# jenkinsm13/julia-spira

Measured on AMD Instinct MI355X. Metric: Msamples/sec at 1920x1080 spp=64 depth=8; fraction of HBM roofline, higher is better.
Workload: dtype f64

## Files before the change

julia-spira_amd/csrc/spira_device.h:

```cpp
#pragma once
#include <hip/hip_runtime.h>
#include <stdint.h>
#include <type_traits>
#include "spira_fastdiv.h"

namespace spira {

__device__ __forceinline__ float sqrt_rn(float x) { return __builtin_sqrtf(x); }
__device__ __forceinline__ double sqrt_rn(double x) { return __builtin_sqrt(x); }

constexpr int kBlock = 256;
#ifndef SPIRA_WAVES_F32
#define SPIRA_WAVES_F32 5
#endif
#ifndef SPIRA_WAVES_F64
#define SPIRA_WAVES_F64 4
#endif
#define SPIRA_WAVES_PER_SIMD(T) (sizeof(T) == 8 ? SPIRA_WAVES_F64 : SPIRA_WAVES_F32)
constexpr uint32_t kMaxTries = 64;

template <class T> struct Vec { T x, y, z; };

template <class T> __device__ __forceinline__ Vec<T> mk(T x, T y, T z) { Vec<T> r; r.x = x; r.y = y; r.z = z; return r; }
template <class T> __device__ __forceinline__ Vec<T> operator+(Vec<T> a, Vec<T> b) { return mk<T>(a.x + b.x, a.y + b.y, a.z + b.z); }
template <class T> __device__ __forceinline__ Vec<T> operator-(Vec<T> a, Vec<T> b) { return mk<T>(a.x - b.x, a.y - b.y, a.z - b.z); }
template <class T> __device__ __forceinline__ Vec<T> operator*(Vec<T> a, T b) { return mk<T>(a.x * b, a.y * b, a.z * b); }
template <class T> __device__ __forceinline__ Vec<T> operator/(Vec<T> a, T b) { return mk<T>(a.x / b, a.y / b, a.z / b); }
template <class T> __device__ __forceinline__ Vec<T> mulv(Vec<T> a, Vec<T> b) { return mk<T>(a.x * b.x, a.y * b.y, a.z * b.z); }
template <class T> __device__ __forceinline__ T dot(Vec<T> a, Vec<T> b) { return a.x * b.x + a.y * b.y + a.z * b.z; }
template <class T> __device__ __forceinline__ Vec<T> cross(Vec<T> a, Vec<T> b) {
    return mk<T>(a.y * b.z - a.z * b.y, a.z * b.x - a.x * b.z, a.x * b.y - a.y * b.x);
}
__device__ __forceinline__ float abs_t(float x) { return __builtin_fabsf(x); }
__device__ __forceinline__ double abs_t(double x) { return __builtin_fabs(x); }
template <class T> __device__ __forceinline__ Vec<T> normalize(Vec<T> a) { return a / sqrt_rn(dot(a, a)); }

struct ExactDiv {};
// ... 691 lines not shown
            oc = o - mk<T>(c.x, c.y, c.z);
            cc = dot(oc, oc) - c.w;
        }
        T b = (T)2.0 * dot(oc, d);
        const T bb = b * b;
        T disc = bb - four_a * cc;
        if (!(disc < 0)) {
            root_operands<T>(bb, disc, pol);
            T sq = root_sqrt<T>(disc, pol);
            T root = root_over<T>(-b - sq, over_2a, pol);
            bool ok = !(root < t_min || root > closest);
            if (!ok && root < t_min) {
                root = root_over<T>(-b + sq, over_2a, pol);
                ok = !(root < t_min || root > closest);
            }
            if (ok) { closest = root; prim = (int)s; }
        }
    }
    if (TRI && sc.n_triangles) {
        Pack4<T> v0n = sc.tri[0], e1n = sc.tri[1], e2n = sc.tri[2];
#pragma unroll 2
        for (uint32_t i = 0; i < sc.n_triangles; ++i) {
            const Pack4<T> v0 = v0n, e1 = e1n, e2 = e2n;
            const uint32_t nx = i + 1 < sc.n_triangles ? i + 1 : i;
            v0n = sc.tri[3 * nx]; e1n = sc.tri[3 * nx + 1]; e2n = sc.tri[3 * nx + 2];
            T t;
            if (triangle_test<T>(v0, e1, e2, o, d, t_min, closest, t, pol)) {
                closest = t; prim = (int)(sc.n_spheres + i);
            }
        }
    }
}

template <class T>
__device__ __forceinline__ bool mesh_box_hit(const SceneLds<T> &sc, Vec<T> o, Vec<T> d, T closest) {
    const Vec<T> inv = mk<T>(rcp_fast(d.x), rcp_fast(d.y), rcp_fast(d.z));
    return box_entry<T>(sc.bvh_root[0], sc.bvh_root[1], o, inv, closest) >= (T)0;
}

template <class T>
__device__ __forceinline__ void closest_hit_local(const SceneLds<T> &sc, Vec<T> o, Vec<T> d, T t_min, T &closest, int &prim) {
    ExactDiv exact;
    closest_hit_local<T>(sc, o, d, t_min, closest, prim, exact);
}
template <class T, bool BVH, class P, bool TRI = true>
__device__ __forceinline__ int closest_hit(const SceneLds<T> &sc, Vec<T> o, Vec<T> d, T t_min, T &t_hit, uint32_t &slot, P &pol) {
    T closest; int prim;
    closest_hit_local<T, P, TRI>(sc, o, d, t_min, closest, prim, pol);
    slot = 0;
    if (BVH) bvh_closest_hit<T>(sc, o, d, t_min, closest, prim, slot);
    t_hit = closest;
    return prim;
}
template <class T, bool BVH>
__device__ __forceinline__ int closest_hit(const SceneLds<T> &sc, Vec<T> o, Vec<T> d, T t_min, T &t_hit, uint32_t &slot) {
    ExactDiv exact;
    return closest_hit<T, BVH>(sc, o, d, t_min, t_hit, slot, exact);
}

template <class T> __device__ __forceinline__ Vec<T> random_in_unit_sphere(const RngKey &k) {
    Vec<T> p = mk<T>(0, 0, 0);
    for (uint32_t t = 1; t <= kMaxTries; ++t) {
        T u0, u1, u2;
        rng3<T>(k, t, u0, u1, u2, (T)(1.0 / 1048576.0));
        Vec<T> q = mk<T>(u0, u1, u2) - mk<T>(1, 1, 1);
        if (dot(q, q) < (T)1.0) { p = q; break; }
// ... 174 lines not shown
                                           Vec<T> &o, Vec<T> &d, P &pol) {
    T xu, xv, unused;
    rng3<T>(rng_key(rc.sA, rc.sB, pixel, sample, 0), 0, xu, xv, unused);
    T u = ((T)(i - 1) + xu) / (T)(rc.width - 1);
    T v = ((T)(j - 1) + xv) / (T)(rc.height - 1);
    o = rc.cam_origin;
    d = normalize(((rc.cam_llc + rc.cam_hor * u) + rc.cam_ver * v) - o, pol);
}
template <class T>
__device__ __forceinline__ void camera_ray(const RenderConst<T> &rc, uint32_t i, uint32_t j, uint32_t pixel, uint32_t sample,
                                           Vec<T> &o, Vec<T> &d) {
    ExactDiv exact;
    camera_ray<T>(rc, i, j, pixel, sample, o, d, exact);
}
__device__ __forceinline__ float to_scalar(float x) { return __uint_as_float(__builtin_amdgcn_readfirstlane(__float_as_uint(x))); }
__device__ __forceinline__ double to_scalar(double x) {
    const uint32_t lo = __builtin_amdgcn_readfirstlane((uint32_t)__double2loint(x)), hi = __builtin_amdgcn_readfirstlane((uint32_t)__double2hiint(x));
    return __hiloint2double((int)hi, (int)lo);
}
template <class T> struct PixelDiv { Recip<T> w1, h1; };
template <class T> __device__ __forceinline__ PixelDiv<T> pixel_divisors(const RenderConst<T> &rc) {
    PixelDiv<T> p;
    p.w1 = recip_of((T)(rc.width - 1)); p.h1 = recip_of((T)(rc.height - 1));
    p.w1.d = to_scalar(p.w1.d); p.w1.r = to_scalar(p.w1.r); p.h1.d = to_scalar(p.h1.d); p.h1.r = to_scalar(p.h1.r);
    return p;
}
template <class T> __device__ __forceinline__ T pixel_quotient(T n, const Recip<T> &rc, ExactDiv &) { return n / rc.d; }
template <class T> __device__ __forceinline__ T pixel_quotient(T n, const Recip<T> &rc, SpecDiv &) { return quotient(n, rc); }
template <class T, class P>
__device__ __forceinline__ void camera_ray_lds(const RenderConst<T> &rc, const T *cam, const PixelDiv<T> &pd, uint32_t i, uint32_t j, uint32_t pixel, uint32_t sample,
                                               Vec<T> &o, Vec<T> &d, P &pol) {
    T xu, xv, unused;
    rng3<T>(rng_key(rc.sA, rc.sB, pixel, sample, 0), 0, xu, xv, unused);
    T u = pixel_quotient<T>((T)(i - 1) + xu, pd.w1, pol);
    T v = pixel_quotient<T>((T)(j - 1) + xv, pd.h1, pol);
    o = mk<T>(cam[0], cam[1], cam[2]);
    const Vec<T> llc = mk<T>(cam[3], cam[4], cam[5]), hor = mk<T>(cam[6], cam[7], cam[8]), ver = mk<T>(cam[9], cam[10], cam[11]);
    d = normalize(((llc + hor * u) + ver * v) - o, pol);
}

template <class T>
__device__ __forceinline__ void path_of(const RenderConst<T> &rc, uint32_t q, uint32_t pass, uint32_t &i, uint32_t &j,
                                        uint32_t &pixel, uint32_t &sample) {
    uint32_t slot = fastdiv(q, rc.fd_tile);
    uint32_t pl = q - slot * rc.tile_pixels;
    uint32_t lr = fastdiv(pl, rc.fd_width);
    uint32_t lx = pl - lr * rc.width;
    j = ref_row_j(rc, lr);
    i = lx + 1;
    pixel = (j - 1) * rc.width + lx;
    sample = rc.sample0 + pass * rc.slots + slot;
}

template <class T> struct RayQueue { Pack4<T> *A; Pack4<T> *B; Pack2<T> *C; };

struct Stats {
    unsigned long long segments, rays_enqueued, radiance_rmw, radiance_store, redone_waves, rays_parked;
    unsigned long long mesh_wave_trips, mesh_lane_trips;
};

template <class T> struct BounceArgs {
    SceneGlobal<T> scene;
    RenderConst<T> rc;
    RayQueue<T> qin, qout;
    Pack3<T> *L;
    const uint32_t *cnt_in;
// ... 245 lines not shown
        a.blk_stats[4 * wid + 1] = n_rmw;
        a.blk_stats[4 * wid + 2] = n_store;
        a.blk_stats[4 * wid + 3] = FIRST ? 0u : n_seg;
    }
}

template <class T> struct PathArgs {
    SceneGlobal<T> scene;
    RenderConst<T> rc;
    RayQueue<T> q[2];
    uint32_t *qref[2];
    uint2 *qkey[2];
    uint32_t cam_consts;
    Pack3<T> *L;
    uint32_t *blk_stats;
    uint32_t cap;
    uint32_t pass;
    uint32_t n_first;
    uint32_t dense_pct;
    Pack4<T> *mesh_list;
    uint32_t mesh_min_batch;
    uint32_t refill_free;
    uint32_t mesh_mode;
    uint32_t *mesh_count;
    uint32_t resume_k, resume_nw;
    uint32_t *redo;
    uint32_t redo_only;
    Stats *stats;
    Pack4<T> *accum;
    FastDiv fd_keff;
    uint32_t k_eff;
    uint32_t accum_first;
    uint32_t l_private;
};

#ifndef SPIRA_RESOLVE_RUN
#define SPIRA_RESOLVE_RUN 4
#endif
__device__ __forceinline__ uint32_t owned_pixel(uint32_t w, uint32_t nw, uint32_t l) {
    constexpr uint32_t kRun = SPIRA_RESOLVE_RUN;
    static_assert(64 % kRun == 0, "a run length divides the wave");
    return ((l / kRun) * nw + w) * kRun + l % kRun;
}

template <class T>
__device__ __forceinline__ void resolve_pixel(Pack4<T> *accum, const Pack3<T> *L, uint32_t tile_pixels, uint32_t k_eff, bool first_pass, uint32_t p) {
    Pack4<T> acc;
    if (first_pass) { acc.x = 0; acc.y = 0; acc.z = 0; acc.w = 0; } else acc = accum[p];
    uint32_t s = 0;
    for (; s + 8 <= k_eff; s += 8) {
        Pack3<T> l[8];
#pragma unroll
        for (int k = 0; k < 8; ++k) l[k] = L[(size_t)(s + k) * tile_pixels + p];
#pragma unroll
        for (int k = 0; k < 8; ++k) { acc.x = acc.x + l[k].x; acc.y = acc.y + l[k].y; acc.z = acc.z + l[k].z; }
    }
    for (; s < k_eff; ++s) {
        const Pack3<T> l = L[(size_t)s * tile_pixels + p];
        acc.x = acc.x + l.x; acc.y = acc.y + l.y; acc.z = acc.z + l.z;
    }
    accum[p] = acc;
}
template <class T>
__device__ __forceinline__ void resolve_pixel_run(Pack4<T> *accum, const Pack3<T> *Lp, uint32_t k_eff, bool first_pass, uint32_t p) {
    constexpr uint32_t kRun = SPIRA_RESOLVE_RUN;
    Pack4<T> acc;
    if (first_pass) { acc.x = 0; acc.y = 0; acc.z = 0; acc.w = 0; } else acc = accum[p];
// ... 64 lines not shown
    constexpr bool kCam = !EXT;
    if (kCam && MODE != 2 && a.cam_consts)
        for (uint32_t i = threadIdx.x; i < a.scene.n_spheres; i += blockDim.x) {
            const T *sp = a.scene.spheres5 + 5 * (size_t)i;
            const Vec<T> oc = rc.cam_origin - mk<T>(sp[0], sp[1], sp[2]);
            Pack4<T> k; k.x = oc.x; k.y = oc.y; k.z = oc.z; k.w = dot(oc, oc) - sp[3] * sp[3];
            cam_sph[i] = k;
        }
    const SceneLds<T> sc = stage_scene<T>(a.scene, lds_raw);
    const PixelDiv<T> pix_div = pixel_divisors<T>(rc);
    if (!SPEC && a.redo_only) {
        if (!a.redo[wid]) return;
        if (lane == 0) atomicAdd(&a.stats->redone_waves, 1ull);
    }
    Pack4<T> *s_rnd = reinterpret_cast<Pack4<T> *>(lds_raw + scene_lds_bytes<T>(a.scene.n_spheres, a.scene.n_materials, a.scene.n_triangles)) + wave * SUB;
    constexpr uint32_t mesh_mode = BVH ? (uint32_t)MODE : 0u;
    const uint32_t kseg = mesh_mode == 2u ? a.resume_k : 1u;
    if (mesh_mode == 2u && wid * kseg >= a.resume_nw) return;
    const uint32_t region = wid * kseg * a.cap;
    const unsigned long long lt_mask = (1ull << lane) - 1ull;
    const uint32_t ref_base = sc.n_spheres + sc.n_triangles;
    const bool mixed = mesh_mode != 0u || rc.max_depth <= 128u;
    const uint32_t dense_pct = mixed ? a.dense_pct : 0u;
    const bool defer = mesh_mode != 0u || (BVH && mixed && a.mesh_list != nullptr);
    Pack4<T> *mlist = a.mesh_list + 3 * (size_t)region;
    uint32_t n_rmw = 0, n_store = 0, n_seg = 0, n_enq = 0, n_park = 0;
    uint32_t n_wtrips = 0, n_ltrips = 0;
    uint32_t n_in = 0;
    const bool own = !BVH && !EXT && !TRI && sizeof(T) == 8 && a.accum != nullptr;
    const uint32_t n_own = own ? 64u * a.k_eff : 0u;
    const uint32_t n_sub_first = own ? (n_own + SUB - 1) / SUB : (a.n_first + SUB - 1) / SUB;
    const bool priv = kCarry && own && a.l_private != 0;
    const uint32_t l_base = priv ? wid * n_own : 0u;

    auto park = [&](uint32_t slot_i, const Vec<T> o_, const Vec<T> d_, const Vec<T> beta_, T closest_, uint32_t q_, int prim_, uint32_t stage_hit) {
        Pack4<T> A, B, C;
        A.x = o_.x; A.y = o_.y; A.z = o_.z; A.w = d_.x;
        B.x = d_.y; B.y = d_.z; B.z = beta_.x; B.w = beta_.y;
        C.x = beta_.z; C.y = closest_; C.z = Bits<T>::from_u32(q_); C.w = Bits<T>::from_u32((uint32_t)(prim_ + 1) | (stage_hit << kStageShift));
        mlist[3 * (size_t)slot_i] = A; mlist[3 * (size_t)slot_i + 1] = B; mlist[3 * (size_t)slot_i + 2] = C;
    };
    uint32_t mfill = 0;
    constexpr int kMaxSeg = 16;
    uint32_t pfx[kMaxSeg + 1];
    bool segmented = false;
    {
        uint32_t cnt = 0;
        if (mesh_mode == 2u && lane < kseg && wid * kseg + lane < a.resume_nw) cnt = a.mesh_count[wid * kseg + lane];
        pfx[0] = 0;
#pragma unroll
        for (int j = 0; j < kMaxSeg; ++j) pfx[j + 1] = pfx[j] + (uint32_t)__builtin_amdgcn_readlane((int)cnt, j);
        if (mesh_mode == 2u) { mfill = pfx[kMaxSeg]; segmented = true; }
    }
    const uint32_t first_sub = own ? 0u : (mesh_mode == 1u ? (wid % a.resume_k) * (NW / a.resume_k) + wid / a.resume_k : wid);
    const uint32_t sub_step = own ? 1u : NW;
    MESH_STAT(unsigned long long dbg_t0 = __builtin_readcyclecounter(); unsigned long long dbg_sess = 0, dbg_walk = 0; uint32_t dbg_ns = 0, dbg_ws = 0, dbg_ls = 0, dbg_rf = 0, dbg_rays = 0, dbg_rounds = 0, dbg_ws1 = 0, dbg_ls1 = 0, dbg_h[4] = {0, 0, 0, 0};)
    for (uint32_t round = 0; ; ++round) {
        MESH_STAT(++dbg_rounds;)
        const bool first = mesh_mode != 2u && round == 0;
        const RayQueue<T> qin = a.q[(round + 1) & 1], qout = a.q[round & 1];
        const uint32_t *rin = a.qref[(round + 1) & 1];
        uint32_t *rout = a.qref[round & 1];
        const uint2 *kin = a.qkey[(round + 1) & 1];
        uint2 *kout = a.qkey[round & 1];
        const uint32_t limit = first ? (own ? n_own : a.n_first) : n_in;
        const uint32_t n_sub = first ? n_sub_first : (n_in + SUB - 1) / SUB;
        uint32_t fill = 0;
        for (uint32_t sub = first ? first_sub : 0u; sub < n_sub; sub += first ? sub_step : 1u) {
            Vec<T> o[R], beta[R];
            Pending<T> pend[R];
            ExtState<T> ex[R];
            uint32_t q[R], ent[R], stg[R], ref[R];
            uint32_t ka[R], kb[R];
            bool valid[R];
#pragma unroll
            for (int r = 0; r < R; ++r) {
                const uint32_t idx = sub * SUB + r * 64 + lane;
                valid[r] = false; stg[r] = round; ref[r] = 0; q[r] = 0; ka[r] = 0; kb[r] = 0;
                pend[r].kind = kDead; pend[r].rough = 0; pend[r].v = mk<T>(0, 0, 0);
                o[r] = mk<T>(0, 0, 0); beta[r] = mk<T>(1, 1, 1);
                bool parked = false; T park_t = 0; int park_prim = -1;
                uint32_t qf = idx;
                bool in = idx < limit;
                if (own && first) {
                    const uint32_t t = idx / SPIRA_RESOLVE_RUN, run = fastdiv(t, a.fd_keff);
                    const uint32_t px = owned_pixel(wid, NW, run * SPIRA_RESOLVE_RUN + idx % SPIRA_RESOLVE_RUN);
                    qf = (t - run * a.k_eff) * rc.tile_pixels + px;
                    in = in && px < rc.tile_pixels;
                }
                const uint32_t ql = priv ? l_base + idx : qf;
                if (in) {
                    if (first) {
                        uint32_t pixel, sample, pi, pj;
                        Vec<T> d;
                        q[r] = ql;
                        path_of<T>(rc, qf, a.pass, pi, pj, pixel, sample);
                        if (kCarry) { ka[r] = mix32(rc.sA + pixel) ^ (sample << 8); kb[r] = mix32(rc.sB ^ pixel) + (sample << 8); }
                        camera_ray_lds<T>(rc, cam_lds, pix_div, pi, pj, pixel, sample, o[r], d, pol);
                        if (EXT) { ex[r].flags = rc.flags; if (rc.flags & kExtSpectral) beta[r] = ext_wavelength<T>(sc, rc.sA, rc.sB, pixel, sample, ex[r]); }
                        T t; uint32_t slot = 0;
                        int prim;
                        if (defer) {
                            if (kCam && a.cam_consts) closest_hit_local<T, Pol, TRI, true>(sc, o[r], d, (T)0.001, t, prim, pol, cam_sph);
                            else closest_hit_local<T, Pol, TRI>(sc, o[r], d, (T)0.001, t, prim, pol);
                            parked = mesh_box_hit<T>(sc, o[r], d, t);
                        } else if (kCam && !BVH && a.cam_consts) { closest_hit_local<T, Pol, TRI, true>(sc, o[r], d, (T)0.001, t, prim, pol, cam_sph); }
                        else prim = closest_hit<T, BVH, Pol, TRI>(sc, o[r], d, (T)0.001, t, slot, pol);
                        ++n_seg;
                        if (parked) { park_t = t; park_prim = prim; pend[r].v = d; }
                        else if (prim < 0) {
                            const Vec<T> c = sky_term_x<T, EXT>(d, beta[r], &ex[r]);
                            Pack3<T> l; l.x = c.x; l.y = c.y; l.z = c.z;
                            a.L[ql] = l;
                            ++n_store;
                        } else {
                            valid[r] = true;
                            o[r] = o[r] + d * t;
                            ref[r] = (BVH && prim >= (int)ref_base) ? ref_base + slot : (uint32_t)prim;
                            pend[r].v = d;
                        }
                    } else {
                        const Pack4<T> A = qin.A[region + idx], B = qin.B[region + idx];
                        const Pack2<T> C = qin.C[region + idx];
                        o[r] = mk<T>(A.x, A.y, A.z);
                        pend[r].v = mk<T>(A.w, B.x, B.y);
                        beta[r] = mk<T>(B.z, B.w, C.x);
                        q[r] = unpack_q(C.y);
                        uint32_t w;
                        if constexpr (kRefArray) w = rin[region + idx]; else w = unpack_ref(C.y);
                        if (mixed) { stg[r] = w >> kStageShift; ref[r] = w & kRefMask; } else ref[r] = w;
                        if (kCarry) { const uint2 k = kin[region + idx]; ka[r] = k.x; kb[r] = k.y; }
                        valid[r] = true;
                    }
                }
                if (defer && first) {
// ... 1199 lines not shown
```

julia-spira_amd/csrc/spira_hip.hip:

```cpp
#include <hip/hip_runtime.h>
#include <sys/mman.h>
#include <rccl/rccl.h>
#include <dlfcn.h>

#include <algorithm>
#include <atomic>
#include <chrono>
#include <cmath>
#include <cstdio>
#include <cstdlib>
#include <cstring>
#include <condition_variable>
#include <mutex>
#include <new>
#include <string>
#include <thread>
#include <vector>

#include "../../include/spira_hip.h"
#include "../../include/spira_spd.h"
#include "spira_device.h"
#include "spira_bvh.h"
#include "spira_validate.h"
#include "spira_plan.h"
// ... 534 lines not shown
        static_assert(SPIRA_SPD_N == spira::kSpdN && SPIRA_SPD_ROWS == spira::kSpdRows, "SPD table shape");
        T host[SPIRA_SPD_ROWS * SPIRA_SPD_N];
        for (int r = 0; r < SPIRA_SPD_ROWS; ++r)
            for (int i = 0; i < SPIRA_SPD_N; ++i) host[r * SPIRA_SPD_N + i] = (T)spira_spd_table[r][i];
        if (int rc = b.ensure(sizeof host)) return rc;
        HIP_TRY(hipMemcpy(b.p, host, sizeof host, hipMemcpyHostToDevice));
    }
    (void)st;
    g.spd = (const T *)b.p;
    return 0;
}

template <class T>
int check_handle(const spira_scene *h) {
    if (!h || h->magic != kSceneMagic) return fail(SPIRA_E_INVALID, "scene handle is NULL or was destroyed");
    if (h->prec != (int)sizeof(T)) return fail(SPIRA_E_INVALID, "scene handle was created in the other precision");
    if (h->device != tl_device) return fail(SPIRA_E_INVALID, "scene handle belongs to another device (spira_set_device)");
    return 0;
}

spira::Knobs read_knobs() {
    spira::Knobs k;
    k.batch_rays = env_u32("SPIRA_BATCH_RAYS", k.batch_rays);
    k.R = env_u32("SPIRA_R", k.R);
    k.blocks_per_cu = env_u32("SPIRA_BLOCKS_PER_CU", 0);
    k.defer_mesh = env_u32("SPIRA_DEFER_MESH", 1); k.mesh_two_pass = env_u32("SPIRA_MESH_TWO_PASS", 1);
    k.fused_resolve = env_u32("SPIRA_FUSED_RESOLVE", 1); k.private_l = env_u32("SPIRA_PRIVATE_L", 1);
    k.spec_div = env_u32("SPIRA_SPEC_DIV", 1);
    k.dense_pct = std::min<uint32_t>(env_u32("SPIRA_DENSE_PCT", 70), 100);
    k.mesh_min_batch = std::max<uint32_t>(1, env_u32("SPIRA_MESH_MIN_BATCH", 128));
    k.mesh_refill = std::min<uint32_t>(64, std::max<uint32_t>(1, env_u32("SPIRA_MESH_REFILL", 16)));
    k.mesh_fat_waves_per_cu = env_u32("SPIRA_MESH_FAT_WAVES_PER_CU", 16);
    k.cam_consts = env_u32("SPIRA_CAM_CONSTS", 1);
    return k;
}
template <class T>
spira::PlanIn plan_input(const Ctx &c, const spira_params *p, uint32_t rows, uint32_t nt_scene, bool progressive, bool caller_rng, bool out_on_device) {
    spira::PlanIn in;
    in.width = p->width; in.rows = rows; in.spp = p->spp; in.max_depth = p->max_depth; in.flags = p->flags; in.batch_rays = p->batch_rays;
    in.n_triangles = nt_scene; in.num_cus = (uint32_t)c.num_cus;
    in.progressive = progressive; in.caller_rng = caller_rng; in.out_on_device = out_on_device;
    in.prec = sizeof(T); in.block = spira::kBlock; in.waves_per_simd = SPIRA_WAVES_PER_SIMD(T); in.carry_key = SPIRA_CARRY_KEY;
    in.pack4 = sizeof(spira::Pack4<T>); in.pack3 = sizeof(spira::Pack3<T>); in.pack2 = sizeof(spira::Pack2<T>);
    in.k = read_knobs();
    return in;
}

int ensure_workspaces(Ctx &c, const spira::Workspace &w) {
    for (int i = 0; i < 2; ++i) {
        if (int rc = c.qA[i].ensure(w.queue4)) return rc;
        if (int rc = c.qB[i].ensure(w.queue4)) return rc;
        if (int rc = c.qC[i].ensure(w.queue2)) return rc;
        if (int rc = c.qR[i].ensure(w.q_ref)) return rc;
        if (int rc = c.qK[i].ensure(w.q_key)) return rc;
        if (int rc = c.qX[i].ensure(w.q_x)) return rc;
    }
    const struct { DevBuf &b; uint64_t bytes; } rest[] = {
        {c.mesh_list, w.mesh_list}, {c.mesh_count, w.mesh_count}, {c.redo, w.redo}, {c.blkstats, w.blkstats}, {c.L, w.L}, {c.counts, w.counts},
        {c.stats, sizeof(spira::Stats)}, {c.accum, w.accum}, {c.out_tmp, w.out_tmp}, {c.rng, w.rng},
        {c.hyb_state, w.hyb_state}, {c.hyb_mat, w.hyb_mat}, {c.hyb_flags, w.hyb_flags}};
    for (const auto &r : rest)
        if (int rc = r.b.ensure(r.bytes)) return rc;
    return 0;
}

template <class T>
int verify_path_args(const Ctx &c, const spira::PathArgs<T> &a, uint32_t first_launch_blocks) {
    using P4 = spira::Pack4<T>;
    using P2 = spira::Pack2<T>;
    spira::PathLaunch l;
    l.blocks = first_launch_blocks; l.cap = a.cap; l.n_first = a.n_first; l.k_eff = a.k_eff;
    l.tile_pixels = a.rc.tile_pixels; l.max_depth = a.rc.max_depth; l.flags = a.rc.flags; l.n_lds_triangles = a.scene.n_triangles;
    l.mesh_mode = a.mesh_mode; l.resume_k = a.resume_k; l.resume_nw = a.resume_nw;
    l.mesh = a.scene.n_bvh_tris != 0; l.pixel_owning = a.accum != nullptr; l.l_private = a.l_private != 0;
    l.prec = sizeof(T); l.wpb = spira::kBlock / 64; l.carry_key = SPIRA_CARRY_KEY;
    const spira::PathNeed need = spira::path_need(l);
    const uint64_t nw = need.nw, n = need.packets;
    auto covers = [](const DevBuf &b, const void *ptr, uint64_t bytes) { return ptr == b.p && b.p != nullptr && b.cap >= bytes; };
    const char *bad = need.fits ? nullptr : "the pass does not fit its queue regions";
    if (a.rc.max_depth > 1 || l.mesh)
        for (int i = 0; i < 2 && !bad; ++i) {
            if (!covers(c.qA[i], a.q[i].A, n * sizeof(P4)) || !covers(c.qB[i], a.q[i].B, n * sizeof(P4)) || !covers(c.qC[i], a.q[i].C, n * sizeof(P2))) bad = "hit queues";
            else if (sizeof(T) == 4 && !covers(c.qR[i], a.qref[i], n * sizeof(uint32_t))) bad = "hit reference arrays";
            else if (!l.mesh && !covers(c.qK[i], a.qkey[i], n * sizeof(uint2))) bad = "carried RNG keys";
        }
    if (!bad && a.mesh_list && !covers(c.mesh_list, a.mesh_list, 3 * n * sizeof(P4))) bad = "mesh lists";
    if (!bad && a.mesh_mode != 0 && (!a.mesh_list || !covers(c.mesh_count, a.mesh_count, nw * sizeof(uint32_t)) || !need.resume_ok)) bad = "parked-ray counts of a two-launch mesh pass";
    if (!bad && a.redo && !covers(c.redo, a.redo, nw * sizeof(uint32_t))) bad = "redo flags";
    if (!bad && !covers(c.blkstats, a.blk_stats, nw * 4 * sizeof(uint32_t))) bad = "per-wave statistics";
    if (!bad && !covers(c.L, a.L, need.l_entries * sizeof(spira::Pack3<T>))) bad = "per-path radiance";
    if (!bad && !covers(c.stats, a.stats, sizeof(spira::Stats))) bad = "counters";
    if (!bad && a.accum && (!covers(c.accum, a.accum, (uint64_t)a.rc.tile_pixels * sizeof(P4)) || !need.owning_ok)) bad = "pixel-owning pass";
    if (!bad && a.l_private && !need.private_ok) bad = "wave-private radiance blocks";
    if (bad) return fail(SPIRA_E_LIMIT, std::string("internal: a workspace is smaller than the launch needs (") + bad + ")");
    return 0;
}

template <class T>
int validate_call(const spira_scene *h, const T *spheres5, const T *materials8, const T *triangles10, const T *camera12, const spira_params *p,
                  const T *out_hdr, const T *out_img, bool progressive, uint32_t sample0, const uint32_t *rng_states, uint32_t *rows) {
    if (!p) return fail(SPIRA_E_INVALID, "params is NULL");
    const uint32_t nt = triangles10 ? p->n_triangles : 0;
    if (h) { if (int rc = check_handle<T>(h)) return rc; }
    else if (int rc = validate_scene<T>(spheres5, materials8, triangles10, p->n_spheres, p->n_materials, nt)) return rc;
    if (int rc = validate_params(camera12, p, h ? h->store.nt : nt, rows)) return rc;
    if (!out_hdr && !out_img) return fail(SPIRA_E_INVALID, "both outputs are NULL");
    const char *msg = nullptr;
    if (int rc = spira::sample_range_check(progressive, sample0, p->spp, &msg)) return fail(rc, msg);
    if (progressive && (p->flags & SPIRA_SEM_MASK) == SPIRA_SEM_HYBRID) return fail(SPIRA_E_UNSUPPORTED, "SPIRA_SEM_HYBRID has no accumulate entry (its image is a mean of tone-mapped samples)");
    if (progressive && (p->flags & SPIRA_SEM_MASK) == SPIRA_SEM_METAL && sample0 > 0 && !rng_states)
        return fail(SPIRA_E_INVALID, "SPIRA_SEM_METAL with sample0 > 0 needs rng_states (the LCG states the previous call left); "
                                     "without them every call would replay the samples of the first");
    return 0;
}

template <class T> struct Call {
    Ctx &c;
    hipStream_t st;
    const spira_params *p;
    const spira::Plan &plan;
    spira::BounceArgs<T> a{};
    size_t lds = 0;
    int spec = 0;
    bool progressive = false, profile = false;
    uint32_t sample0 = 0, *d_rng = nullptr;
    uint64_t launches = 0, metal_launches = 0;
// ... 105 lines not shown
    const spira::Plan &plan = k.plan;
    const spira::Knobs &kn = plan.in.k;
    spira::PathArgs<T> pa{};
    pa.scene = k.a.scene; pa.rc = k.a.rc; pa.L = k.a.L; pa.pass = k.a.pass; pa.n_first = k.a.n_first;
    pa.dense_pct = kn.dense_pct;
    pa.mesh_list = plan.defer_mesh ? (P4 *)c.mesh_list.p : nullptr;
    const spira::Geometry g = plan.geometry(pa.n_first);
    const uint32_t G = g.G;
    pa.cap = g.cap;
    *stat_rows = G * plan.wpb;
    for (int i = 0; i < 2; ++i) {
        pa.q[i] = k.queue(i);
        pa.qref[i] = (uint32_t *)c.qR[i].p;
        pa.qkey[i] = (uint2 *)c.qK[i].p;
    }
    pa.blk_stats = (uint32_t *)c.blkstats.p;
    pa.stats = k.stats();
    if (k.spec) pa.redo = k.redo();
    pa.mesh_mode = 0; pa.mesh_count = nullptr; pa.resume_k = 1; pa.resume_nw = 0;
    pa.mesh_min_batch = kn.mesh_min_batch;
    pa.refill_free = kn.mesh_refill;
    size_t lds_a = k.lds + (size_t)plan.wpb * plan.sub * sizeof(P4) + 128;
    pa.cam_consts = (kn.cam_consts && pa.scene.n_spheres && lds_a + (size_t)pa.scene.n_spheres * sizeof(P4) <= (size_t)160 * 1024) ? 1u : 0u;
    if (pa.cam_consts) lds_a += (size_t)pa.scene.n_spheres * sizeof(P4);
    if (plan.two_pass) {
        pa.mesh_mode = 1; pa.mesh_count = (uint32_t *)c.mesh_count.p;
        pa.resume_nw = G * plan.wpb; pa.resume_k = plan.fat_k(pa.resume_nw);
    }
    if (plan.fused) {
        pa.accum = k.accum(); pa.k_eff = plan.k_eff(pa.pass); pa.fd_keff = spira::fastdiv_make(pa.k_eff);
        pa.accum_first = (pa.pass == 0 && !k.progressive) ? 1u : 0u;
        pa.l_private = plan.l_private ? 1u : 0u;
    }
    if (int rc = verify_path_args<T>(c, pa, G)) return rc;
    HIP_TRY(hipEventRecord(c.ev_pool[c.ev_used++], k.st));
    if (int rc = launch_path<T>((int)plan.R, dim3(G), lds_a, k.st, pa, k.spec)) return rc;
    if (int rc = lds_optin_failed()) return rc;
    k.launches += k.spec ? 2 : 1;
    if (pa.mesh_mode == 1) {
        if (c.ev_mid.size() <= c.ev_mid_used) {
            hipEvent_t e;
            HIP_TRY(hipEventCreate(&e));
            c.ev_mid.push_back(e); c.ev_mid_end.push_back(0);
        }
        HIP_TRY(hipEventRecord(c.ev_mid[c.ev_mid_used], k.st));
        c.ev_mid_end[c.ev_mid_used++] = c.ev_used;
        spira::PathArgs<T> pb = pa;
        pb.mesh_mode = 2; pb.n_first = 0;
        const uint32_t nwb = pa.resume_nw / pa.resume_k;
        launch_path_resume_entry<T>((int)plan.R, dim3((nwb + plan.wpb - 1) / plan.wpb), lds_a, k.st, pb);
        if (int rc = lds_optin_failed()) return rc;
        ++k.launches;
    }
    HIP_TRY(hipEventRecord(c.ev_pool[c.ev_used++], k.st));
    return 0;
}

template <class T>
int enqueue_bounce_pass(Call<T> &k, uint32_t *stat_rows) {
    using P4 = typename Call<T>::P4;
    Ctx &c = k.c;
    const spira::Plan &plan = k.plan;
    const spira::Geometry g = plan.geometry(k.a.n_first);
    const size_t nw = (size_t)g.G * plan.wpb;
    k.a.cap = g.cap;
    *stat_rows = k.p->max_depth * g.G * plan.wpb;
    for (uint32_t b = 0; b < k.p->max_depth; ++b) {
// ... 1247 lines not shown
```

julia-spira_amd/csrc/spira_plan.h:

```cpp
#pragma once
#include <algorithm>
#include <cstdint>

#include "../../include/spira_hip.h"

namespace spira {

struct Knobs {
    uint32_t batch_rays = 160u << 20;
    uint32_t R = 2;
    uint32_t blocks_per_cu = 0;
    uint32_t defer_mesh = 1, mesh_two_pass = 1, fused_resolve = 1, private_l = 1;
    uint32_t spec_div = 1;
    uint32_t dense_pct = 70, mesh_min_batch = 128, mesh_refill = 16, mesh_fat_waves_per_cu = 16, cam_consts = 1;
};

struct PlanIn {
    uint32_t width = 0, rows = 0;
    uint32_t spp = 0, max_depth = 0, flags = 0, batch_rays = 0;
    uint32_t n_triangles = 0;
    uint32_t num_cus = 0;
    bool progressive = false, caller_rng = false, out_on_device = false;
    bool adaptive = false;
    uint32_t prec = 0, block = 0, waves_per_simd = 0, carry_key = 0;
    uint32_t pack4 = 0, pack3 = 0, pack2 = 0;
    Knobs k;
};

enum class Org { Black, Hybrid, MetalWavefront, Metal, Cpu, Mega, Path, Bounce };

struct Geometry { uint32_t G, cap; };

struct Workspace {
    uint64_t queue4 = 0, queue2 = 0, q_ref = 0, q_key = 0, q_x = 0;
    uint64_t mesh_list = 0, mesh_count = 0, redo = 0, blkstats = 0, L = 0, counts = 0, accum = 0, out_tmp = 0, rng = 0;
    uint64_t hyb_state = 0, hyb_mat = 0, hyb_flags = 0;
};

struct Plan {
    PlanIn in;
    Org org = Org::Black;
    uint32_t R = 2, wpb = 0, sub = 0, max_blocks = 0;
    uint64_t tile_pixels = 0, batch = 0;
    uint32_t slots = 0, n_pass = 0;
    bool mesh_scene = false, defer_mesh = false, two_pass = false;
    bool fused = false, l_private = false;
    bool spec_allowed = false;
    uint32_t G_max = 0, cap_max = 0;
    uint64_t q_rays = 0;
    uint32_t ppw = 0, G_metal = 0;
    Workspace ws;

    Geometry geometry(uint64_t n_first) const {
        if (fused) {
            const uint64_t k = n_first / tile_pixels;
            return {(uint32_t)((tile_pixels + 64 * wpb - 1) / (64 * wpb)), (uint32_t)((64 * k + sub - 1) / sub * sub)};
        }
        const uint64_t n_sub = (n_first + sub - 1) / sub;
        const uint32_t G = (uint32_t)std::min<uint64_t>((n_sub + wpb - 1) / wpb, max_blocks);
        const uint64_t nw = (uint64_t)G * wpb;
        return {G, (uint32_t)(((n_sub + nw - 1) / nw) * sub)};
    }
    uint32_t k_eff(uint32_t pass) const { return std::min(slots, in.spp - pass * slots); }
    uint32_t n_first(uint32_t pass) const { return (uint32_t)((uint64_t)k_eff(pass) * tile_pixels); }
    uint32_t blocks(uint64_t n) const { return (uint32_t)std::min<uint64_t>((n + in.block - 1) / in.block, max_blocks); }
    uint32_t fat_k(uint32_t nw) const {
        const uint32_t fat = std::max<uint32_t>(1, in.num_cus * in.k.mesh_fat_waves_per_cu);
        uint32_t k = 16;
        while (k > 1 && (nw % k != 0 || nw / k < fat)) k >>= 1;
        return k;
    }
    int spec(bool moderate) const {
        uint32_t s = spec_allowed ? in.k.spec_div : 0;
        if (s == 1 && !moderate) s = 0;
        return s > 2 ? 1 : (int)s;
    }
};

inline int sample_range_check(bool progressive, uint32_t sample0, uint32_t spp, const char **msg) {
    if (progressive && (uint64_t)sample0 + spp > SPIRA_MAX_SPP) { *msg = "sample0 + spp exceeds 2^24"; return SPIRA_E_LIMIT; }
    return 0;
}

inline int make_plan(const PlanIn &in, Plan &pl, const char **msg) {
    auto bad = [&](const char *m) { *msg = m; return SPIRA_E_LIMIT; };
    pl = Plan{};
    pl.in = in;
    const Knobs &k = in.k;
    const uint32_t sem = in.flags & SPIRA_SEM_MASK, kern = in.flags & SPIRA_KERNEL_MASK;
    const bool ext = (in.flags & (SPIRA_EXT_DIELECTRIC | SPIRA_EXT_SPECTRAL)) != 0;
    const uint64_t tp = pl.tile_pixels = (uint64_t)in.rows * in.width;
    const uint32_t target = in.batch_rays ? in.batch_rays : k.batch_rays;
    uint64_t slots = std::min<uint64_t>(std::max<uint64_t>(1, target / tp), in.spp);
    const uint64_t n_pass = (in.spp + slots - 1) / slots;
    slots = (in.spp + n_pass - 1) / n_pass;
    if (slots * tp > 0x7FFFFFFFull) return bad("tile too large: rows*width must be < 2^31");
    pl.slots = (uint32_t)slots;
    pl.n_pass = (in.spp + pl.slots - 1) / pl.slots;
    pl.batch = slots * tp;
    pl.org = sem == SPIRA_SEM_HYBRID ? Org::Hybrid : sem == SPIRA_SEM_METAL ? (kern == SPIRA_KERNEL_WAVEFRONT ? Org::MetalWavefront : Org::Metal) :
             sem == SPIRA_SEM_CPU ? Org::Cpu : kern == SPIRA_KERNEL_MEGA ? Org::Mega : kern == SPIRA_KERNEL_BOUNCE ? Org::Bounce : Org::Path;
    const bool persistent = pl.org == Org::Path;
    pl.R = (k.R == 1 && !ext) ? 1 : 2;
    pl.mesh_scene = in.n_triangles > SPIRA_LDS_TRIANGLES;
    pl.defer_mesh = persistent && pl.mesh_scene && in.max_depth <= 128 && k.defer_mesh != 0;
    pl.two_pass = pl.defer_mesh && k.mesh_two_pass != 0;

    const uint32_t blocks_per_cu = k.blocks_per_cu ? k.blocks_per_cu : !persistent ? 16 : (pl.mesh_scene && !pl.two_pass) ? 4 : 32;
    pl.max_blocks = (uint32_t)std::min<uint64_t>((uint64_t)in.num_cus * blocks_per_cu, 0x7FFFFFFFull);
    pl.wpb = in.block / 64;
    pl.sub = 64 * pl.R;
    pl.fused = persistent && in.prec == 8 && pl.R == 2 && in.n_triangles == 0 && !ext && pl.slots <= 64 && k.fused_resolve != 0 && !in.adaptive;
    const Geometry g = pl.geometry(pl.batch);
    pl.G_max = g.G; pl.cap_max = g.cap;
    const uint64_t waves = (uint64_t)g.G * pl.wpb;
    pl.l_private = pl.fused && in.carry_key && in.max_depth <= 128 && k.private_l != 0 && 64ull * waves * pl.slots <= 0x7FFFFFFFull;
    pl.q_rays = (uint64_t)g.cap * waves;
    if (pl.q_rays > 0xFFFFFFFFull) return bad("pass too large");
    pl.spec_allowed = pl.org == Org::Cpu || (pl.org == Org::Metal && !in.progressive) || (pl.org == Org::MetalWavefront && !in.progressive && pl.R == 2) ||
                      (persistent && pl.R == 2);
    if (in.max_depth == 0) pl.org = Org::Black;

    Workspace &w = pl.ws;
    const uint64_t redo_per_wave = (pl.spec_allowed && k.spec_div) ? sizeof(uint32_t) : 0, stat_row = 4 * sizeof(uint32_t);
    w.accum = tp * in.pack4;
    w.out_tmp = in.out_on_device ? 0 : 2 * 3 * tp * in.prec;
    if (in.caller_rng && !in.out_on_device) w.rng = tp * sizeof(uint32_t);
    switch (pl.org) {
    case Org::Black: break;
    case Org::Hybrid:
        if (tp > 0xFFFFFFFFull / 2) return bad("image too large for SPIRA_SEM_HYBRID");
        w.hyb_state = 12 * tp * in.prec; w.hyb_mat = w.rng = tp * sizeof(uint32_t);
        w.hyb_flags = (uint64_t)in.spp * (in.max_depth + 1) * sizeof(uint32_t);
        break;
    case Org::MetalWavefront: {
        const uint64_t nw0 = (uint64_t)in.num_cus * in.waves_per_simd * pl.wpb;
        pl.ppw = (uint32_t)((((tp + nw0 - 1) / nw0) + 63) / 64 * 64);
        pl.G_metal = (uint32_t)((tp + (uint64_t)pl.ppw * pl.wpb - 1) / ((uint64_t)pl.ppw * pl.wpb));
        const uint64_t nw = (uint64_t)pl.G_metal * pl.wpb, n = nw * pl.ppw;
        w.queue4 = n * in.pack4; w.queue2 = n * in.pack2; w.q_x = n * 2 * sizeof(uint32_t); w.L = n * in.pack3;
        if (!in.caller_rng) w.rng = tp * sizeof(uint32_t);
        w.blkstats = nw * stat_row; w.redo = nw * redo_per_wave;
        break;
    }
    case Org::Metal: case Org::Cpu: case Org::Mega:
        w.L = pl.batch * in.pack3; w.blkstats = waves * stat_row;
        w.redo = (pl.org == Org::Metal ? pl.blocks(tp) : pl.org == Org::Cpu ? pl.max_blocks : 0) * (uint64_t)pl.wpb * redo_per_wave;
        break;
    case Org::Bounce:
        if (in.max_depth > 1) { w.queue4 = pl.q_rays * in.pack4; w.queue2 = pl.q_rays * in.pack2; }
        w.L = pl.batch * in.pack3;
        w.counts = (uint64_t)(in.max_depth + 2) * waves * sizeof(uint32_t); w.blkstats = (uint64_t)(in.max_depth + 1) * waves * stat_row;
        break;
    case Org::Path:
        if (in.max_depth > 1 || pl.mesh_scene) {
            w.queue4 = pl.q_rays * in.pack4; w.queue2 = pl.q_rays * in.pack2;
            if (in.prec == 4) w.q_ref = pl.q_rays * sizeof(uint32_t);
            if (!pl.defer_mesh) w.q_key = pl.q_rays * 2 * sizeof(uint32_t);
        }
        if (pl.defer_mesh) w.mesh_list = 3 * pl.q_rays * in.pack4;
        if (pl.two_pass) w.mesh_count = waves * sizeof(uint32_t);
        w.redo = waves * redo_per_wave; w.blkstats = waves * stat_row;
        w.L = (pl.l_private ? std::max<uint64_t>(pl.batch, 64ull * waves * pl.slots) : pl.batch) * in.pack3;
        break;
    }
    return 0;
}

struct PathLaunch {
    uint32_t blocks = 0, cap = 0, n_first = 0, k_eff = 0;
    uint32_t tile_pixels = 0, max_depth = 0, flags = 0, n_lds_triangles = 0;
    uint32_t mesh_mode = 0, resume_k = 1, resume_nw = 0;
    bool mesh = false, pixel_owning = false, l_private = false;
    uint32_t prec = 0, wpb = 0, carry_key = 0;
};
struct PathNeed {
    uint64_t nw, packets, l_entries;
    bool fits, resume_ok, owning_ok, private_ok;
};
inline PathNeed path_need(const PathLaunch &a) {
    PathNeed n{};
    n.nw = (uint64_t)a.blocks * a.wpb;
    n.packets = n.nw * a.cap;
    n.fits = a.n_first <= n.packets;
    n.resume_ok = a.resume_k != 0 && a.resume_k <= 16 && n.nw % a.resume_k == 0 && a.resume_nw == n.nw;
    n.l_entries = a.l_private ? std::max<uint64_t>(a.n_first, 64ull * n.nw * a.k_eff) : a.n_first;
    const uint64_t tp = a.tile_pixels;
    n.owning_ok = a.prec == 8 && !a.n_lds_triangles && !a.mesh && !(a.flags & (SPIRA_EXT_DIELECTRIC | SPIRA_EXT_SPECTRAL)) && a.k_eff != 0 && a.k_eff <= 64 &&
                  (uint64_t)a.k_eff * tp == a.n_first && 64 * n.nw >= tp && a.cap >= 64ull * a.k_eff;
    n.private_ok = a.pixel_owning && a.carry_key && a.max_depth <= 128 && n.l_entries <= 0x80000000ull;
    return n;
}

struct AdaptiveIn {
    uint32_t min_spp = 0, batch_spp = 0, spp = 0;
    double tolerance = 0, floor = 0;
    uint64_t tile_pixels = 0;
    uint32_t prec = 0, pack3 = 0, num_cus = 0;
};
constexpr uint32_t kAdaptiveItems = 256, kAdaptiveWpb = 4;
struct AdaptiveRound { uint32_t samples, chunk, ppw, grid; uint64_t waves; };
struct AdaptivePlan {
    AdaptiveIn in;
    uint32_t levels = 0;
    uint64_t list_cap = 0;
    uint64_t list_bytes = 0, q_bytes = 0, n_bytes = 0, count_bytes = 0;
    uint64_t lds_round = 0;
    uint32_t level(uint32_t r) const { return (uint32_t)std::min<uint64_t>((uint64_t)in.min_spp + (uint64_t)r * in.batch_spp, in.spp); }
    AdaptiveRound round(uint32_t r, uint64_t n_active) const {
        AdaptiveRound a{};
        a.samples = level(r) - level(r - 1);
        a.chunk = std::min(a.samples, kAdaptiveItems);
        const uint64_t want_waves = std::max<uint64_t>(1, (uint64_t)in.num_cus * 16);
        const uint64_t spread = (n_active + want_waves - 1) / want_waves;
        a.ppw = (uint32_t)std::max<uint64_t>(1, std::min<uint64_t>(std::min<uint32_t>(64, kAdaptiveItems / a.chunk), spread));
        a.waves = (n_active + a.ppw - 1) / a.ppw;
        a.grid = (uint32_t)((a.waves + kAdaptiveWpb - 1) / kAdaptiveWpb);
        return a;
    }
};
inline int adaptive_check(uint32_t min_spp, uint32_t batch_spp, uint32_t spp, double tolerance, double floor, const char **msg) {
    if (min_spp < 2) { *msg = "spira_adaptive: min_spp must be >= 2 (a variance needs two samples)"; return SPIRA_E_INVALID; }
    if (batch_spp < 1) { *msg = "spira_adaptive: batch_spp must be >= 1"; return SPIRA_E_INVALID; }
// ... 85 lines not shown
```

Measured before the change: 28160.

## Add per-wave LDS pixel table and camera-ray sphere culling masks

In the fused pixel-owning f64 path, each wave precomputes per-lane pixel coordinates and RNG hash constants into an LDS table. This removes the repeated path_of divisions and hashing for every primary ray. It also builds a conservative per-pixel-footprint bitmask of spheres that camera rays could hit, and primary rays test only those spheres. The cost is extra LDS per block, a setup loop over spheres per lane, and the risk that a culling bound that is not conservative enough drops hits.

```diff
diff --git a/julia-spira_amd/csrc/spira_cam_cull.h b/julia-spira_amd/csrc/spira_cam_cull.h
--- /dev/null
+++ b/julia-spira_amd/csrc/spira_cam_cull.h
@@ -0,0 +1,40 @@
+#pragma once
+#include <math.h>
+#include <stdint.h>
+#if defined(__HIPCC__)
+#define SPIRA_CULL_HD __host__ __device__
+#else
+#define SPIRA_CULL_HD
+#endif
+
+namespace spira {
+
+constexpr uint32_t kPixelTableEntry = 16, kPixelTableWave = 64 * kPixelTableEntry + 64 * 8;
+constexpr uint32_t kCamCullMaxSpheres = 64;
+
+SPIRA_CULL_HD inline bool cam_sphere_culled(const double *cam, uint32_t W, uint32_t H, uint32_t pi, uint32_t pj, const double *pk) {
+    if (W < 2 || H < 2) return false;
+    const double kMargin = 1.0 / 1073741824.0;
+    const double ocx = pk[0], ocy = pk[1], ocz = pk[2];
+    const double oc2 = ocx * ocx + ocy * ocy + ocz * ocz;
+    const double slack = kMargin * oc2;
+    if (!(pk[3] > slack)) return false;
+    const double r2 = oc2 - pk[3];
+    const double w1 = (double)(W - 1), h1 = (double)(H - 1);
+    const double uc = ((double)pi - 0.5) / w1, vc = ((double)pj - 0.5) / h1;
+    const double hu = 0.5 / w1, hv = 0.5 / h1;
+    const double dcx = (cam[3] + cam[6] * uc + cam[9] * vc) - cam[0];
+    const double dcy = (cam[4] + cam[7] * uc + cam[10] * vc) - cam[1];
+    const double dcz = (cam[5] + cam[8] * uc + cam[11] * vc) - cam[2];
+    const double rho = hu * sqrt(cam[6] * cam[6] + cam[7] * cam[7] + cam[8] * cam[8]) + hv * sqrt(cam[9] * cam[9] + cam[10] * cam[10] + cam[11] * cam[11]);
+    const double cx = ocy * dcz - ocz * dcy, cy = ocz * dcx - ocx * dcz, cz = ocx * dcy - ocy * dcx;
+    const double N = sqrt(cx * cx + cy * cy + cz * cz) - sqrt(oc2) * rho;
+    const double M = sqrt(dcx * dcx + dcy * dcy + dcz * dcz) + rho;
+    if (!(N > 0)) return false;
+    const double lhs = N * N, rhs = (r2 + slack) * (M * M);
+    if (!(lhs > rhs)) return false;
+    const double fin = lhs + rhs;
+    return fin - fin == 0;
+}
+
+}
diff --git a/julia-spira_amd/csrc/spira_device.h b/julia-spira_amd/csrc/spira_device.h
--- a/julia-spira_amd/csrc/spira_device.h
+++ b/julia-spira_amd/csrc/spira_device.h
@@ -3,6 +3,7 @@
 #include <stdint.h>
 #include <type_traits>
 #include "spira_fastdiv.h"
+#include "spira_cam_cull.h"
 
 namespace spira {
 
@@ -760,6 +761,43 @@
     }
 }
 
+template <class T, class P>
+__device__ __forceinline__ void closest_hit_cam_masked(Vec<T> d, T t_min, T &closest, int &prim, P &pol, const Pack4<T> *cam, unsigned long long mask) {
+    closest = (T)INFINITY;
+    prim = -1;
+    const T a = dot(d, d);
+    const T two_a = (T)2.0 * a;
+    const T four_a = (T)4 * a;
+    const RootDiv<T> over_2a = root_divisor<T>(two_a, pol);
+    root_t_min<T>(t_min, pol);
+    if (!mask) return;
+    uint32_t s_next = (uint32_t)__builtin_ctzll(mask);
+    mask &= mask - 1ull;
+    Pack4<T> c_next = cam[s_next];
+    while (true) {
+        const Pack4<T> c = c_next;
+        const uint32_t s = s_next;
+        const bool more = mask != 0;
+        if (more) { s_next = (uint32_t)__builtin_ctzll(mask); mask &= mask - 1ull; c_next = cam[s_next]; }
+        const Vec<T> oc = mk<T>(c.x, c.y, c.z);
+        T b = (T)2.0 * dot(oc, d);
+        const T bb = b * b;
+        T disc = bb - four_a * c.w;
+        if (!(disc < 0)) {
+            root_operands<T>(bb, disc, pol);
+            T sq = root_sqrt<T>(disc, pol);
+            T root = root_over<T>(-b - sq, over_2a, pol);
+            bool ok = !(root < t_min || root > closest);
+            if (!ok && root < t_min) {
+                root = root_over<T>(-b + sq, over_2a, pol);
+                ok = !(root < t_min || root > closest);
+            }
+            if (ok) { closest = root; prim = (int)s; }
+        }
+        if (!more) break;
+    }
+}
+
 template <class T>
 __device__ __forceinline__ bool mesh_box_hit(const SceneLds<T> &sc, Vec<T> o, Vec<T> d, T closest) {
     const Vec<T> inv = mk<T>(rcp_fast(d.x), rcp_fast(d.y), rcp_fast(d.z));
@@ -1000,6 +1038,19 @@
                                                Vec<T> &o, Vec<T> &d, P &pol) {
     T xu, xv, unused;
     rng3<T>(rng_key(rc.sA, rc.sB, pixel, sample, 0), 0, xu, xv, unused);
+    T u = pixel_quotient<T>((T)(i - 1) + xu, pd.w1, pol);
+    T v = pixel_quotient<T>((T)(j - 1) + xv, pd.h1, pol);
+    o = mk<T>(cam[0], cam[1], cam[2]);
+    const Vec<T> llc = mk<T>(cam[3], cam[4], cam[5]), hor = mk<T>(cam[6], cam[7], cam[8]), ver = mk<T>(cam[9], cam[10], cam[11]);
+    d = normalize(((llc + hor * u) + ver * v) - o, pol);
+}
+template <class T, class P>
+__device__ __forceinline__ void camera_ray_lds(const T *cam, const PixelDiv<T> &pd, uint32_t i, uint32_t j, uint32_t mA, uint32_t mB, uint32_t sample,
+                                               Vec<T> &o, Vec<T> &d, P &pol) {
+    T xu, xv, unused;
+    RngKey k;
+    k.hA = mix32(mA ^ (sample << 8)); k.hB = mix32(mB + (sample << 8)); k.hBr = (k.hB << 16) | (k.hB >> 16);
+    rng3<T>(k, 0, xu, xv, unused);
     T u = pixel_quotient<T>((T)(i - 1) + xu, pd.w1, pol);
     T v = pixel_quotient<T>((T)(j - 1) + xv, pd.h1, pol);
     o = mk<T>(cam[0], cam[1], cam[2]);
@@ -1311,7 +1362,9 @@
     uint32_t k_eff;
     uint32_t accum_first;
     uint32_t l_private;
+    uint32_t pixel_table;
 };
+constexpr uint32_t kTableConsts = 1u, kTableCull = 2u;
 
 #ifndef SPIRA_RESOLVE_RUN
 #define SPIRA_RESOLVE_RUN 4
@@ -1442,6 +1495,38 @@
     const uint32_t n_sub_first = own ? (n_own + SUB - 1) / SUB : (a.n_first + SUB - 1) / SUB;
     const bool priv = kCarry && own && a.l_private != 0;
     const uint32_t l_base = priv ? wid * n_own : 0u;
+    constexpr bool kOwn = !BVH && !EXT && !TRI && sizeof(T) == 8 && R == 2 && MODE == 0;
+    uint32_t tab_bits = 0;
+    const uint4 *ptab = nullptr;
+    const uint2 *pmask = nullptr;
+    if constexpr (kOwn) {
+        if (own && a.pixel_table) {
+            constexpr uint32_t kRun = SPIRA_RESOLVE_RUN;
+            tab_bits = a.pixel_table;
+            unsigned char *tb = reinterpret_cast<unsigned char *>(cam_sph + (a.cam_consts ? a.scene.n_spheres : 0u)) +
+                                (uint32_t)__builtin_amdgcn_readfirstlane((int)wave) * kPixelTableWave;
+            uint4 *tab_w = reinterpret_cast<uint4 *>(tb);
+            uint2 *mask_w = reinterpret_cast<uint2 *>(tb + 64 * kPixelTableEntry);
+            const uint32_t px = owned_pixel(wid, NW, lane);
+            uint4 e = make_uint4(0u, 0u, 0u, 0u);
+            unsigned long long m = 0;
+            if (px < rc.tile_pixels) {
+                uint32_t pi, pj, pixel, sample;
+                path_of<T>(rc, px, a.pass, pi, pj, pixel, sample);
+                e = make_uint4(pi, pj, mix32(rc.sA + pixel), mix32(rc.sB ^ pixel));
+                if (tab_bits & kTableCull)
+                    for (uint32_t s = 0; s < a.scene.n_spheres; ++s)
+                        if (!cam_sphere_culled(cam_lds, rc.width, rc.height, pi, pj, &cam_sph[s].x)) m |= 1ull << s;
+            }
+            uint32_t lo = (uint32_t)m, hi = (uint32_t)(m >> 32);
+#pragma unroll
+            for (uint32_t dl = 1; dl < kRun; dl <<= 1) { lo |= (uint32_t)__shfl_xor((int)lo, (int)dl); hi |= (uint32_t)__shfl_xor((int)hi, (int)dl); }
+            tab_w[lane] = e;
+            if (lane % kRun == 0) mask_w[lane / kRun] = make_uint2(lo, hi);
+            wave_lds_sync();
+            ptab = tab_w; pmask = mask_w;
+        }
+    }
 
     auto park = [&](uint32_t slot_i, const Vec<T> o_, const Vec<T> d_, const Vec<T> beta_, T closest_, uint32_t q_, int prim_, uint32_t stage_hit) {
         Pack4<T> A, B, C;
@@ -1492,11 +1577,38 @@
                 bool parked = false; T park_t = 0; int park_prim = -1;
                 uint32_t qf = idx;
                 bool in = idx < limit;
+                uint4 pe = make_uint4(0u, 0u, 0u, 0u);
+                uint32_t own_slot = 0;
+                unsigned long long cmask = 0;
                 if (own && first) {
                     const uint32_t t = idx / SPIRA_RESOLVE_RUN, run = fastdiv(t, a.fd_keff);
-                    const uint32_t px = owned_pixel(wid, NW, run * SPIRA_RESOLVE_RUN + idx % SPIRA_RESOLVE_RUN);
-                    qf = (t - run * a.k_eff) * rc.tile_pixels + px;
-                    in = in && px < rc.tile_pixels;
+                    bool from_table = false;
+                    if constexpr (kOwn) {
+                        if (tab_bits & kTableConsts) {
+                            const uint32_t l = (run * SPIRA_RESOLVE_RUN + idx % SPIRA_RESOLVE_RUN) & 63u;
+                            pe = ptab[l];
+                            own_slot = t - run * a.k_eff;
+                            in = in && pe.x != 0u;
+                            if (!priv) qf = own_slot * rc.tile_pixels + owned_pixel(wid, NW, l);
+                            from_table = true;
+                        }
+                        if (tab_bits & kTableCull) {
+                            constexpr uint32_t kLastRun = 64u / SPIRA_RESOLVE_RUN - 1u;
+                            const uint32_t i0 = sub * SUB + r * 64;
+                            const uint32_t run0 = min(fastdiv(i0 / SPIRA_RESOLVE_RUN, a.fd_keff), kLastRun);
+                            const uint32_t run1 = min(fastdiv((i0 + 63u) / SPIRA_RESOLVE_RUN, a.fd_keff), kLastRun);
+                            for (uint32_t rn = run0; rn <= run1; ++rn) {
+                                const uint2 mm = pmask[rn];
+                                cmask |= (unsigned long long)(uint32_t)__builtin_amdgcn_readfirstlane((int)mm.x) |
+                                         ((unsigned long long)(uint32_t)__builtin_amdgcn_readfirstlane((int)mm.y) << 32);
+                            }
+                        }
+                    }
+                    if (!from_table) {
+                        const uint32_t px = owned_pixel(wid, NW, run * SPIRA_RESOLVE_RUN + idx % SPIRA_RESOLVE_RUN);
+                        qf = (t - run * a.k_eff) * rc.tile_pixels + px;
+                        in = in && px < rc.tile_pixels;
+                    }
                 }
                 const uint32_t ql = priv ? l_base + idx : qf;
                 if (in) {
@@ -1504,13 +1616,29 @@
                         uint32_t pixel, sample, pi, pj;
                         Vec<T> d;
                         q[r] = ql;
-                        path_of<T>(rc, qf, a.pass, pi, pj, pixel, sample);
-                        if (kCarry) { ka[r] = mix32(rc.sA + pixel) ^ (sample << 8); kb[r] = mix32(rc.sB ^ pixel) + (sample << 8); }
-                        camera_ray_lds<T>(rc, cam_lds, pix_div, pi, pj, pixel, sample, o[r], d, pol);
+                        bool from_table = false;
+                        if constexpr (kOwn) {
+                            if (tab_bits & kTableConsts) {
+                                sample = rc.sample0 + a.pass * rc.slots + own_slot;
+                                ka[r] = pe.z ^ (sample << 8); kb[r] = pe.w + (sample << 8);
+                                camera_ray_lds<T>(cam_lds, pix_div, pe.x, pe.y, pe.z, pe.w, sample, o[r], d, pol);
+                                from_table = true;
+                            }
+                        }
+                        if (!from_table) {
+                            path_of<T>(rc, qf, a.pass, pi, pj, pixel, sample);
+                            if (kCarry) { ka[r] = mix32(rc.sA + pixel) ^ (sample << 8); kb[r] = mix32(rc.sB ^ pixel) + (sample << 8); }
+                            camera_ray_lds<T>(rc, cam_lds, pix_div, pi, pj, pixel, sample, o[r], d, pol);
+                        }
                         if (EXT) { ex[r].flags = rc.flags; if (rc.flags & kExtSpectral) beta[r] = ext_wavelength<T>(sc, rc.sA, rc.sB, pixel, sample, ex[r]); }
                         T t; uint32_t slot = 0;
                         int prim;
-                        if (defer) {
+                        bool scanned = false;
+                        if constexpr (kOwn) {
+                            if (tab_bits & kTableCull) { closest_hit_cam_masked<T, Pol>(d, (T)0.001, t, prim, pol, cam_sph, cmask); scanned = true; }
+                        }
+                        if (scanned) {}
+                        else if (defer) {
                             if (kCam && a.cam_consts) closest_hit_local<T, Pol, TRI, true>(sc, o[r], d, (T)0.001, t, prim, pol, cam_sph);
                             else closest_hit_local<T, Pol, TRI>(sc, o[r], d, (T)0.001, t, prim, pol);
                             parked = mesh_box_hit<T>(sc, o[r], d, t);
diff --git a/julia-spira_amd/csrc/spira_hip.hip b/julia-spira_amd/csrc/spira_hip.hip
--- a/julia-spira_amd/csrc/spira_hip.hip
+++ b/julia-spira_amd/csrc/spira_hip.hip
@@ -590,6 +590,7 @@
     k.mesh_refill = std::min<uint32_t>(64, std::max<uint32_t>(1, env_u32("SPIRA_MESH_REFILL", 16)));
     k.mesh_fat_waves_per_cu = env_u32("SPIRA_MESH_FAT_WAVES_PER_CU", 16);
     k.cam_consts = env_u32("SPIRA_CAM_CONSTS", 1);
+    k.pixel_table = env_u32("SPIRA_PIXEL_TABLE", 1); k.cam_cull = env_u32("SPIRA_CAM_CULL", 1);
     return k;
 }
 template <class T>
@@ -623,7 +624,7 @@
 }
 
 template <class T>
-int verify_path_args(const Ctx &c, const spira::PathArgs<T> &a, uint32_t first_launch_blocks) {
+int verify_path_args(const Ctx &c, const spira::PathArgs<T> &a, uint32_t first_launch_blocks, size_t lds_table_at, size_t lds_launch) {
     using P4 = spira::Pack4<T>;
     using P2 = spira::Pack2<T>;
     spira::PathLaunch l;
@@ -632,6 +633,7 @@
     l.mesh_mode = a.mesh_mode; l.resume_k = a.resume_k; l.resume_nw = a.resume_nw;
     l.mesh = a.scene.n_bvh_tris != 0; l.pixel_owning = a.accum != nullptr; l.l_private = a.l_private != 0;
     l.prec = sizeof(T); l.wpb = spira::kBlock / 64; l.carry_key = SPIRA_CARRY_KEY;
+    l.pixel_table = a.pixel_table; l.n_spheres = a.scene.n_spheres; l.cam_consts = a.cam_consts; l.lds_table_at = lds_table_at; l.lds_launch = lds_launch;
     const spira::PathNeed need = spira::path_need(l);
     const uint64_t nw = need.nw, n = need.packets;
     auto covers = [](const DevBuf &b, const void *ptr, uint64_t bytes) { return ptr == b.p && b.p != nullptr && b.cap >= bytes; };
@@ -650,6 +652,7 @@
     if (!bad && !covers(c.stats, a.stats, sizeof(spira::Stats))) bad = "counters";
     if (!bad && a.accum && (!covers(c.accum, a.accum, (uint64_t)a.rc.tile_pixels * sizeof(P4)) || !need.owning_ok)) bad = "pixel-owning pass";
     if (!bad && a.l_private && !need.private_ok) bad = "wave-private radiance blocks";
+    if (!bad && !need.table_ok) bad = "pixel tables";
     if (bad) return fail(SPIRA_E_LIMIT, std::string("internal: a workspace is smaller than the launch needs (") + bad + ")");
     return 0;
 }
@@ -821,7 +824,13 @@
         pa.accum_first = (pa.pass == 0 && !k.progressive) ? 1u : 0u;
         pa.l_private = plan.l_private ? 1u : 0u;
     }
-    if (int rc = verify_path_args<T>(c, pa, G)) return rc;
+    const size_t lds_table_at = lds_a;
+    if (plan.table_lds() && lds_a + plan.table_lds() <= (size_t)160 * 1024) {
+        pa.pixel_table = (plan.table_consts ? spira::kTableConsts : 0u) |
+                         ((plan.table_cull && pa.cam_consts && pa.scene.n_spheres <= spira::kCamCullMaxSpheres) ? spira::kTableCull : 0u);
+        if (pa.pixel_table) lds_a += plan.table_lds();
+    }
+    if (int rc = verify_path_args<T>(c, pa, G, lds_table_at, lds_a)) return rc;
     HIP_TRY(hipEventRecord(c.ev_pool[c.ev_used++], k.st));
     if (int rc = launch_path<T>((int)plan.R, dim3(G), lds_a, k.st, pa, k.spec)) return rc;
     if (int rc = lds_optin_failed()) return rc;
diff --git a/julia-spira_amd/csrc/spira_plan.h b/julia-spira_amd/csrc/spira_plan.h
--- a/julia-spira_amd/csrc/spira_plan.h
+++ b/julia-spira_amd/csrc/spira_plan.h
@@ -3,6 +3,7 @@
 #include <cstdint>
 
 #include "../../include/spira_hip.h"
+#include "spira_cam_cull.h"
 
 namespace spira {
 
@@ -13,6 +14,7 @@
     uint32_t defer_mesh = 1, mesh_two_pass = 1, fused_resolve = 1, private_l = 1;
     uint32_t spec_div = 1;
     uint32_t dense_pct = 70, mesh_min_batch = 128, mesh_refill = 16, mesh_fat_waves_per_cu = 16, cam_consts = 1;
+    uint32_t pixel_table = 1, cam_cull = 1;
 };
 
 struct PlanIn {
@@ -45,6 +47,7 @@
     uint32_t slots = 0, n_pass = 0;
     bool mesh_scene = false, defer_mesh = false, two_pass = false;
     bool fused = false, l_private = false;
+    bool table_consts = false, table_cull = false;
     bool spec_allowed = false;
     uint32_t G_max = 0, cap_max = 0;
     uint64_t q_rays = 0;
@@ -61,6 +64,7 @@
         const uint64_t nw = (uint64_t)G * wpb;
         return {G, (uint32_t)(((n_sub + nw - 1) / nw) * sub)};
     }
+    uint32_t table_lds() const { return (table_consts || table_cull) ? wpb * kPixelTableWave : 0; }
     uint32_t k_eff(uint32_t pass) const { return std::min(slots, in.spp - pass * slots); }
     uint32_t n_first(uint32_t pass) const { return (uint32_t)((uint64_t)k_eff(pass) * tile_pixels); }
     uint32_t blocks(uint64_t n) const { return (uint32_t)std::min<uint64_t>((n + in.block - 1) / in.block, max_blocks); }
@@ -111,6 +115,8 @@
     pl.wpb = in.block / 64;
     pl.sub = 64 * pl.R;
     pl.fused = persistent && in.prec == 8 && pl.R == 2 && in.n_triangles == 0 && !ext && pl.slots <= 64 && k.fused_resolve != 0 && !in.adaptive;
+    pl.table_consts = pl.fused && k.pixel_table != 0;
+    pl.table_cull = pl.fused && k.cam_cull != 0;
     const Geometry g = pl.geometry(pl.batch);
     pl.G_max = g.G; pl.cap_max = g.cap;
     const uint64_t waves = (uint64_t)g.G * pl.wpb;
@@ -173,10 +179,14 @@
     uint32_t mesh_mode = 0, resume_k = 1, resume_nw = 0;
     bool mesh = false, pixel_owning = false, l_private = false;
     uint32_t prec = 0, wpb = 0, carry_key = 0;
+    uint32_t pixel_table = 0, n_spheres = 0, cam_consts = 0;
+    uint64_t lds_table_at = 0, lds_launch = 0;
 };
 struct PathNeed {
     uint64_t nw, packets, l_entries;
     bool fits, resume_ok, owning_ok, private_ok;
+    uint64_t lds_table;
+    bool table_ok;
 };
 inline PathNeed path_need(const PathLaunch &a) {
     PathNeed n{};
@@ -189,6 +199,10 @@
     n.owning_ok = a.prec == 8 && !a.n_lds_triangles && !a.mesh && !(a.flags & (SPIRA_EXT_DIELECTRIC | SPIRA_EXT_SPECTRAL)) && a.k_eff != 0 && a.k_eff <= 64 &&
                   (uint64_t)a.k_eff * tp == a.n_first && 64 * n.nw >= tp && a.cap >= 64ull * a.k_eff;
     n.private_ok = a.pixel_owning && a.carry_key && a.max_depth <= 128 && n.l_entries <= 0x80000000ull;
+    n.lds_table = a.pixel_table ? (uint64_t)a.wpb * kPixelTableWave : 0;
+    n.table_ok = !a.pixel_table || (a.pixel_owning && a.pixel_table <= 3 && a.lds_table_at % 16 == 0 && a.lds_table_at + n.lds_table <= a.lds_launch &&
+                                    a.lds_launch <= 160ull * 1024 &&
+                                    (!(a.pixel_table & 2u) || (a.cam_consts != 0 && a.n_spheres >= 1 && a.n_spheres <= kCamCullMaxSpheres)));
     return n;
 }
 
```

After: 28450, median of 6. +1.0%, better.
